# haesungpyun/seoul_tourism_recommendation_NGCF

Measured on AMD Instinct MI355X. Metric: NGCF 3-layer forward: propagated edges/sec + achieved HBM GB/s, d=128, higher is better.
Workload: dtype f32

## Files before the change

seoul_tourism_recommendation_ngcf_amd/csrc/common.h:

```cpp
#ifndef NGCF_COMMON_H
#define NGCF_COMMON_H

#include <hip/hip_runtime.h>

#include <algorithm>
#include <cstdarg>
#include <cstdint>
#include <cstdio>
#include <cstdlib>
#include <cstring>
#include <numeric>
#include <thread>
#include <vector>

#include "../../include/ngcf_hip.h"

inline thread_local char g_err[512] = "";

inline int fail(int code, const char *fmt, ...)
{
    va_list ap;
    va_start(ap, fmt);
    vsnprintf(g_err, sizeof(g_err), fmt, ap);
    va_end(ap);
    return code;
}

#define HIP_TRY(expr)                                                                          \
    do {                                                                                       \
        hipError_t e_ = (expr);                                                                \
        if (e_ != hipSuccess)                                                                  \
            return fail(NGCF_ERR_HIP, "%s failed: %s (%s:%d)", #expr, hipGetErrorString(e_),   \
                        __FILE__, __LINE__);                                                   \
    } while (0)

#define LAUNCH_CHECK()                                                                         \
    do {                                                                                       \
        hipError_t e_ = hipGetLastError();                                                     \
        if (e_ != hipSuccess)                                                                  \
            return fail(NGCF_ERR_HIP, "kernel launch failed: %s (%s:%d)", hipGetErrorString(e_), \
                        __FILE__, __LINE__);                                                   \
    } while (0)


struct NgcfOptions {
    int no_fork = 0;
    int no_slicing = 0;
    int no_ldstab = 0;
    int no_panel_split = 0;
    int no_tail_table = 0;
    int no_pad_product = 0;
    int64_t fork_min = 200000000;
    int dense_direct = 1;
    int dense_resident = 1;
    int dense_resident_min_rows = 106496;
    int dense_small_tiles = 1;
    int dense_tall = 1;
    int dense_il_lab = 0;
    int t_rows_bitmap = 1;
    int bwd_input_resident = 1;
    int slice_max_mb = 48;
    int swept_lpe = 16;
    int swept_waves = 0;
    int swept_cut = 4;
    int swept_no_moments = 0;
    int swept_order_rows = 0;
    int swept_debug = 0;
    int swept_window_kb = 0;
    int swept_spin = 500;
    int swept_lead = -2;
    int swept_sync_every = 1;
    int swept_prio_kb = 256;
    int swept_prio_graded = 1;
    int swept_nt = 0;
    int swept_merge = 0;
    char swept_trace[480] = "";
};
extern NgcfOptions g_opts;
const NgcfOptions &ngcf_opts();


constexpr int kMaxDevices = 64;
inline int current_device_slot()
{
    int dev = 0;
    if (hipGetDevice(&dev) != hipSuccess || dev < 0) dev = 0;
    return dev % kMaxDevices;
}

inline int64_t align_up(int64_t x, int64_t a) { return (x + a - 1) / a * a; }
inline bool aligned16(const void *p) { return (reinterpret_cast<uintptr_t>(p) & 15) == 0; }


inline int grid_for(int64_t n, int block)

{
    int64_t g = (n + block - 1) / block;
    if (g < 1) g = 1;
    if (g > 256 * 16) g = 256 * 16;
    return (int)g;
}



struct ngcf_csr {
    int64_t n_rows = 0, n_cols = 0, nnz = 0;
    int64_t max_row_len = 0;
    int64_t *rowptr = nullptr;
    int32_t *colidx = nullptr;
    float *vals = nullptr;
    bool owns = false;
    int64_t cap = 0, pos_len = 0;
    int32_t *pos = nullptr;
    int32_t *scan_blk = nullptr;
    bool borrows_plan = false;
    const struct ngcf_csr *filter_src = nullptr;
    int32_t seg_len = 0;
    int64_t n_seg = 0, n_heavy = 0;
    int32_t *seg_row = nullptr;
    int64_t *seg_begin = nullptr;
    int32_t *heavy_row = nullptr;
    int64_t *heavy_seg_ptr = nullptr;
    struct RowGroup {
        int64_t begin, end;
        bool sliceable;
        int32_t col_lo, col_hi;
        bool lds_table = false;
    };
    std::vector<RowGroup> groups;
    int mode = 0;
    struct SegSet {
        int64_t n_seg = 0, n_heavy = 0;
        int32_t *seg_row = nullptr;
        int64_t *seg_begin = nullptr;
        int32_t *heavy_row = nullptr;
        int64_t *heavy_seg_ptr = nullptr;
    };
    struct Swept {
        struct Part {
            int64_t row_lo = 0, row_hi = 0;
            int waves = 0, rows_per_wave = 0;
            int lpe = 16;
            int32_t n_rowpass = 0, n_win = 0, win_cols = 0, col_lo = 0, col_hi = 0;
            int64_t n_slots = 0, n_partial = 0, n_heavy = 0, partial_base = 0;
            int64_t *tptr = nullptr;
            int32_t *e_pack = nullptr;
            float *e_val = nullptr;
            int32_t *dst = nullptr;
            int32_t *prow = nullptr;
            int32_t *heavy_row = nullptr;
            int64_t *heavy_seg_ptr = nullptr;
        };
        std::vector<Part> parts;
        std::vector<char> group_swept;
        SegSet out;
        int64_t n_partial = 0;
        uint32_t *barrier = nullptr;
        mutable hipStream_t barrier_owner[4] = {nullptr, nullptr, nullptr, nullptr};
        mutable int barrier_used = 0;
        int built_mode = 0;
        int lpe = 16;
    } swept;
};


static const int32_t kLdsTableRows = 512;
static const int32_t kDefaultSegLen = 2048;
static inline int32_t default_seg_len(int64_t nnz)
{
    int32_t s = 64;
    while (s < kDefaultSegLen && (int64_t)s * 4096 < nnz) s *= 2;
    return s;
}

void free_swept(ngcf_csr *c);
int build_swept_plan(ngcf_csr *c, hipStream_t stream);
bool swept_usable(const ngcf_csr *c, int64_t ldE, int d);
void prof_mark(hipStream_t stream, int which);

__device__ inline uint32_t mix32(uint64_t x)
{
    x ^= x >> 33;
    x *= 0xff51afd7ed558ccdULL;
    x ^= x >> 33;
    x *= 0xc4ceb9fe1a85ec53ULL;
    x ^= x >> 33;
    return (uint32_t)x;
}

constexpr uint64_t kSeedPtrTag = 0xD5EDull;
__device__ inline uint64_t resolve_seed(uint64_t s)
{
    if ((s >> 48) == kSeedPtrTag) s = *reinterpret_cast<const uint64_t *>(s & 0xFFFFFFFFFFFFull);
    const uint32_t lo = __builtin_amdgcn_readfirstlane((uint32_t)s), hi = __builtin_amdgcn_readfirstlane((uint32_t)(s >> 32));
    return ((uint64_t)hi << 32) | lo;
}

struct EdgeDrop {
    int n;
    uint32_t thr;
    uint64_t seed[4];
    int transposed;
};

struct EdgeDropR {
    int n;
    uint32_t thr;
// ... 100 lines not shown
```

seoul_tourism_recommendation_ngcf_amd/csrc/dense.hip:

```cpp
#include "common.h"
#include <type_traits>

#ifndef NGCF_DC
#define NGCF_DC 16
#endif
#define NGCF_KC (2 * NGCF_DC)

typedef float f32x16 __attribute__((ext_vector_type(16)));
typedef float f32x4 __attribute__((ext_vector_type(4)));

__global__ __launch_bounds__(256) void pack_weights_kernel(const float *__restrict__ W1, const float *__restrict__ b1,
                                                           const float *__restrict__ W2, const float *__restrict__ b2, int d_in,
                                                           int d_out, int n_chunks, int DOP, int NT, float *__restrict__ Wt,
                                                           float *__restrict__ bias2)
{
    __shared__ float tile[NGCF_KC][33];
    const int groups = DOP / 32;
    const int chunk = blockIdx.x / groups, g = blockIdx.x % groups;
    for (int idx = threadIdx.x; idx < 32 * NGCF_KC; idx += 256) {
        const int w = idx / NGCF_KC, kl = idx % NGCF_KC;
        const int within = g * 32 + w;
        const int t = within % NT, j = (within / NT) % 32, cw = within / (NT * 32);
        const int oc = (cw * NT + t) * 32 + j;
        const int col = chunk * NGCF_DC + (kl % NGCF_DC);
// ... 230 lines not shown
#pragma unroll
        for (int r = 0; r < 16; ++r) {
            const int lr = rw * 32 + (r & 3) + 8 * (r >> 2) + 4 * lh;
            float s = 0.f;
#pragma unroll
            for (int q = 0; q < CW; ++q) s += ssq[lr * CW + q];
            rowss[r] = s;
        }
    }
    if (row0 + BM <= n_rows && d_out == WCOLS) {
#pragma unroll
        for (int r = 0; r < 16; ++r) {
            const int64_t grow = row0 + rw * 32 + (r & 3) + 8 * (r >> 2) + 4 * lh;
            const float inv = 1.f / fmaxf(sqrtf(rowss[r]), 1e-12f);
            float *nrow = norm + grow * ldn + cw * NT * 32 + li;
#pragma unroll
            for (int t = 0; t < NT; ++t) nrow[t * 32] = acc[t][r] * inv;
        }
        if (carry) {
#pragma unroll
            for (int r = 0; r < 16; ++r) {
                const int64_t grow = row0 + rw * 32 + (r & 3) + 8 * (r >> 2) + 4 * lh;
                float *crow = carry + grow * ldc + cw * NT * 32 + li;
#pragma unroll
                for (int t = 0; t < NT; ++t) crow[t * 32] = acc[t][r];
            }
        }
        return;
    }
#pragma unroll
    for (int r = 0; r < 16; ++r) {
        const int64_t grow = row0 + rw * 32 + (r & 3) + 8 * (r >> 2) + 4 * lh;
        if (grow >= n_rows) continue;
        const float nrm = fmaxf(sqrtf(rowss[r]), 1e-12f);
        const float inv = 1.f / nrm;
#pragma unroll
        for (int t = 0; t < NT; ++t) {
            const int col = (cw * NT + t) * 32 + li;
            if (col < d_out) {
                const float v = acc[t][r];
                if (carry) carry[grow * ldc + col] = v;
                norm[grow * ldn + col] = v * inv;
            }
        }
    }
}

constexpr int kResWaves = 8, kResWGs = 256;

__global__ __launch_bounds__(kResWaves * 64) void layer_dense_resident_kernel(
    const float *__restrict__ LE, int64_t ldLE, const float *__restrict__ Es, int64_t ldE, int64_t n_rows, int d_in, int d_out,
    const float *__restrict__ Wt, const float *__restrict__ bias2, int n_chunks, float leaky, float drop_p, uint64_t drop_seed_in,
    const float *__restrict__ drop_mask, int64_t ldm, float *__restrict__ carry, int64_t ldc, float *__restrict__ norm, int64_t ldn)
{
    const uint64_t drop_seed = drop_p > 0.f ? resolve_seed(drop_seed_in) : drop_seed_in;
    constexpr int NT = 4, WCOLS = 128;
    extern __shared__ float Wres[];
    const int tid = threadIdx.x, wave = tid >> 6, lane = tid & 63;
    const int li = lane & 31, lh = lane >> 5;
    {
        const f32x4 *src = reinterpret_cast<const f32x4 *>(Wt);
        f32x4 *dst = reinterpret_cast<f32x4 *>(Wres);
        const int n4 = n_chunks * NGCF_KC * WCOLS / 4;
        for (int i = tid; i < n4; i += kResWaves * 64) dst[i] = src[i];
    }
    __syncthreads();
    const int64_t n_tiles = (n_rows + 31) / 32;
    const int d4 = (d_in + 3) & ~3;
    const float *W = Wres + li * NT;
    float bz[NT];
#pragma unroll
    for (int t = 0; t < NT; ++t) bz[t] = bias2[t * 32 + li];
    const int last = n_chunks - 1;
    const int64_t tile_step = (int64_t)gridDim.x * kResWaves;
    auto row_of = [&](int64_t t) {
        int64_t g = t * 32 + li;
        return g < n_rows ? g : n_rows - 1;
    };
    auto fetch = [&](const float *le_row, const float *e_row, int c, f32x4 &la, f32x4 &lb, f32x4 &ea, f32x4 &eb) {
        const int ca = c * NGCF_DC + lh * 4, cb = ca + 8;
        const int cca = ca < d4 ? ca : d4 - 4, ccb = cb < d4 ? cb : d4 - 4;
        la = *reinterpret_cast<const f32x4 *>(le_row + cca);
        ea = *reinterpret_cast<const f32x4 *>(e_row + cca);
        lb = *reinterpret_cast<const f32x4 *>(le_row + ccb);
        eb = *reinterpret_cast<const f32x4 *>(e_row + ccb);
    };
    f32x4 la0, lb0, ea0, eb0, la1, lb1, ea1, eb1;
    int64_t tile = (int64_t)blockIdx.x * kResWaves + wave;
    {
        const int64_t g0 = row_of(tile < n_tiles ? tile : 0);
        fetch(LE + g0 * ldLE, Es + g0 * ldE, 0, la0, lb0, ea0, eb0);
        fetch(LE + g0 * ldLE, Es + g0 * ldE, last < 1 ? last : 1, la1, lb1, ea1, eb1);
    }
    for (; tile < n_tiles; tile += tile_step) {
        const int64_t row0 = tile * 32;
        const int64_t grow_l = row_of(tile);
        const float *le_row = LE + grow_l * ldLE, *e_row = Es + grow_l * ldE;
        f32x16 acc[NT];
#pragma unroll
        for (int t = 0; t < NT; ++t)
#pragma unroll
            for (int r = 0; r < 16; ++r) acc[t][r] = 0.f;
        auto form = [&](int c, f32x4 la, f32x4 lb, f32x4 ea, f32x4 eb, f32x4 (&a4)[4]) {
            const int ca = c * NGCF_DC + lh * 4, cb = ca + 8;
            if (cb + 4 > d_in) {
#pragma unroll
                for (int q = 0; q < 4; ++q) {
                    if (ca + q >= d_in) la[q] = 0.f, ea[q] = 0.f;
                    if (cb + q >= d_in) lb[q] = 0.f, eb[q] = 0.f;
                }
            }
            a4[0] = la + ea, a4[1] = lb + eb, a4[2] = la * ea, a4[3] = lb * eb;
        };
        auto chunk_mfma = [&](int c, const f32x4 (&a4)[4]) {
            const float *wc = W + (int64_t)c * NGCF_KC * WCOLS;
#pragma unroll
            for (int kb = 0; kb < 4; ++kb) {
#pragma unroll
                for (int sx = 0; sx < 4; ++sx) {
                    const f32x4 bv = *reinterpret_cast<const f32x4 *>(wc + (kb * 8 + lh * 4 + sx) * WCOLS);
                    acc[0] = __builtin_amdgcn_mfma_f32_32x32x2f32(a4[kb][sx], bv.x, acc[0], 0, 0, 0);
                    acc[1] = __builtin_amdgcn_mfma_f32_32x32x2f32(a4[kb][sx], bv.y, acc[1], 0, 0, 0);
                    acc[2] = __builtin_amdgcn_mfma_f32_32x32x2f32(a4[kb][sx], bv.z, acc[2], 0, 0, 0);
                    acc[3] = __builtin_amdgcn_mfma_f32_32x32x2f32(a4[kb][sx], bv.w, acc[3], 0, 0, 0);
                }
            }
        };
        int c = 0;
        for (; c + 1 < n_chunks; c += 2) {
            {
                f32x4 a4[4];
                form(c, la0, lb0, ea0, eb0, a4);
                fetch(le_row, e_row, c + 2 < last ? c + 2 : last, la0, lb0, ea0, eb0);
                __builtin_amdgcn_sched_barrier(0);
                chunk_mfma(c, a4);
            }
            {
                f32x4 a4[4];
                form(c + 1, la1, lb1, ea1, eb1, a4);
                fetch(le_row, e_row, c + 3 < last ? c + 3 : last, la1, lb1, ea1, eb1);
                __builtin_amdgcn_sched_barrier(0);
                chunk_mfma(c + 1, a4);
            }
        }
        if (c < n_chunks) {
            f32x4 a4[4];
            form(c, la0, lb0, ea0, eb0, a4);
            chunk_mfma(c, a4);
        }
        {
            const int64_t gn = row_of(tile + tile_step < n_tiles ? tile + tile_step : tile);
            fetch(LE + gn * ldLE, Es + gn * ldE, 0, la0, lb0, ea0, eb0);
            fetch(LE + gn * ldLE, Es + gn * ldE, last < 1 ? last : 1, la1, lb1, ea1, eb1);
            __builtin_amdgcn_sched_barrier(0);
        }
        const float keep_scale = drop_p > 0.f ? 1.f / (1.f - drop_p) : 1.f;
        const uint32_t drop_thr = drop_p > 0.f ? (uint32_t)((double)drop_p * 4294967296.0) : 0u;
        float rowss[16];
#pragma unroll
        for (int r = 0; r < 16; ++r) rowss[r] = 0.f;
        const bool any_drop = drop_mask || drop_p > 0.f;
        if (!any_drop) {
#pragma unroll
            for (int t = 0; t < NT; ++t)
#pragma unroll
                for (int r = 0; r < 16; ++r) {
                    float v = acc[t][r] + bz[t];
                    v = v >= 0.f ? v : leaky * v;
                    acc[t][r] = v;
                    rowss[r] = fmaf(v, v, rowss[r]);
                }
        } else {
#pragma unroll
            for (int t = 0; t < NT; ++t) {
                const int col = t * 32 + li;
#pragma unroll
                for (int r = 0; r < 16; ++r) {
                    float v = acc[t][r] + bz[t];
                    v = v >= 0.f ? v : leaky * v;
                    const int64_t grow = row0 + (r & 3) + 8 * (r >> 2) + 4 * lh;
                    if (drop_mask) v *= (grow < n_rows && col < d_out) ? drop_mask[grow * ldm + col] : 0.f;
                    else {
                        const uint32_t h = mix32(drop_seed ^ ((uint64_t)grow * 0x9E3779B97F4A7C15ULL + (uint64_t)col));
                        v = h < drop_thr ? 0.f : v * keep_scale;
                    }
                    acc[t][r] = v;
                    rowss[r] = fmaf(v, v, rowss[r]);
                }
            }
        }
#pragma unroll
        for (int r = 0; r < 16; ++r) {
            float s2 = rowss[r];
            s2 += __shfl_xor(s2, 1);
            s2 += __shfl_xor(s2, 2);
            s2 += __shfl_xor(s2, 4);
            s2 += __shfl_xor(s2, 8);
            s2 += __shfl_xor(s2, 16);
            rowss[r] = s2;
        }
        if (row0 + 32 <= n_rows && d_out == WCOLS) {
#pragma unroll
            for (int r = 0; r < 16; ++r) {
                const int64_t grow = row0 + (r & 3) + 8 * (r >> 2) + 4 * lh;
                const float inv = 1.f / fmaxf(sqrtf(rowss[r]), 1e-12f);
                float *nrow = norm + grow * ldn + li;
#pragma unroll
                for (int t = 0; t < NT; ++t) nrow[t * 32] = acc[t][r] * inv;
            }
            if (carry) {
#pragma unroll
                for (int r = 0; r < 16; ++r) {
                    float *crow = carry + (row0 + (r & 3) + 8 * (r >> 2) + 4 * lh) * ldc + li;
#pragma unroll
                    for (int t = 0; t < NT; ++t) crow[t * 32] = acc[t][r];
                }
            }
            continue;
        }
#pragma unroll
        for (int r = 0; r < 16; ++r) {
            const int64_t grow = row0 + (r & 3) + 8 * (r >> 2) + 4 * lh;
            if (grow >= n_rows) continue;
            const float inv = 1.f / fmaxf(sqrtf(rowss[r]), 1e-12f);
#pragma unroll
            for (int t = 0; t < NT; ++t) {
                const int col = t * 32 + li;
                if (col < d_out) {
                    const float v = acc[t][r];
                    if (carry) carry[grow * ldc + col] = v;
                    norm[grow * ldn + col] = v * inv;
                }
            }
        }
    }
}

#ifdef NGCF_LAB
__global__ __launch_bounds__(kResWaves * 64) void layer_dense_resident2_kernel(
    const float *__restrict__ LE, int64_t ldLE, const float *__restrict__ Es, int64_t ldE, int64_t n_rows, int d_in, int d_out,
    const float *__restrict__ Wt, const float *__restrict__ bias2, int n_chunks, float leaky, float drop_p, uint64_t drop_seed_in,
    const float *__restrict__ drop_mask, int64_t ldm, float *__restrict__ carry, int64_t ldc, float *__restrict__ norm, int64_t ldn)
{
    const uint64_t drop_seed = drop_p > 0.f ? resolve_seed(drop_seed_in) : drop_seed_in;
    constexpr int NT = 4, WCOLS = 128, TP = 2;
    extern __shared__ float Wres[];
    const int tid = threadIdx.x, wave = tid >> 6, lane = tid & 63;
    const int li = lane & 31, lh = lane >> 5;
    {
        const f32x4 *src = reinterpret_cast<const f32x4 *>(Wt);
        f32x4 *dst = reinterpret_cast<f32x4 *>(Wres);
        const int n4 = n_chunks * NGCF_KC * WCOLS / 4;
        for (int i = tid; i < n4; i += kResWaves * 64) dst[i] = src[i];
    }
    __syncthreads();
    const int64_t n_pairs = (n_rows + 32 * TP - 1) / (32 * TP);
    const int d4 = (d_in + 3) & ~3;
    const float *W = Wres + li * NT + lh * 4 * WCOLS;
    float bz[NT];
#pragma unroll
    for (int t = 0; t < NT; ++t) bz[t] = bias2[t * 32 + li];
    const int last = n_chunks - 1;
    const int64_t pair_step = (int64_t)gridDim.x * kResWaves;
    auto row_of = [&](int64_t pr, int u) {
        int64_t g = pr * (32 * TP) + u * 32 + li;
        return g < n_rows ? g : n_rows - 1;
    };
    auto fetch = [&](const float *le_row, const float *e_row, int c, f32x4 &la, f32x4 &lb, f32x4 &ea, f32x4 &eb) {
        const int ca = c * NGCF_DC + lh * 4, cb = ca + 8;
        const int cca = ca < d4 ? ca : d4 - 4, ccb = cb < d4 ? cb : d4 - 4;
        la = *reinterpret_cast<const f32x4 *>(le_row + cca);
        ea = *reinterpret_cast<const f32x4 *>(e_row + cca);
        lb = *reinterpret_cast<const f32x4 *>(le_row + ccb);
        eb = *reinterpret_cast<const f32x4 *>(e_row + ccb);
    };
    f32x4 la[TP], lb[TP], ea[TP], eb[TP];
    int64_t pair = (int64_t)blockIdx.x * kResWaves + wave;
#pragma unroll
    for (int u = 0; u < TP; ++u) {
        const int64_t g0 = row_of(pair < n_pairs ? pair : 0, u);
        fetch(LE + g0 * ldLE, Es + g0 * ldE, 0, la[u], lb[u], ea[u], eb[u]);
    }
    for (; pair < n_pairs; pair += pair_step) {
        const int64_t row0 = pair * (32 * TP);
        const float *le_row[TP], *e_row[TP];
#pragma unroll
        for (int u = 0; u < TP; ++u) {
            const int64_t g = row_of(pair, u);
            le_row[u] = LE + g * ldLE, e_row[u] = Es + g * ldE;
        }
        f32x16 acc[TP][NT];
#pragma unroll
        for (int u = 0; u < TP; ++u)
#pragma unroll
            for (int t = 0; t < NT; ++t)
#pragma unroll
                for (int r = 0; r < 16; ++r) acc[u][t][r] = 0.f;
        for (int c = 0; c < n_chunks; ++c) {
            f32x4 a4[TP][4];
            const int ca = c * NGCF_DC + lh * 4, cb = ca + 8;
#pragma unroll
            for (int u = 0; u < TP; ++u) {
                if (cb + 4 > d_in) {
#pragma unroll
                    for (int q = 0; q < 4; ++q) {
                        if (ca + q >= d_in) la[u][q] = 0.f, ea[u][q] = 0.f;
// ... 583 lines not shown
#pragma unroll
        for (int kb = 0; kb < 4; ++kb) b[kb] = *reinterpret_cast<const f32x4 *>(w + kb * 256);
    };
    f32x16 acc[MT];
#pragma unroll
    for (int m = 0; m < MT; ++m)
#pragma unroll
        for (int r = 0; r < 16; ++r) acc[m][r] = 0.f;
    const float *xs_r = Xs + li * XLD + lh * 4;
    auto read_a = [&](int buf, int kb, f32x4 (&a)[MT]) {
#pragma unroll
        for (int m = 0; m < MT; ++m)
            a[m] = *reinterpret_cast<const f32x4 *>(xs_r + buf * XBUF + m * 32 * XLD + (kb >> 1) * NGCF_DC + (kb & 1) * 8);
    };
    auto cl = [&](int c) { return c < last ? c : last; };
    f32x4 an[MT];
    auto step = [&](int c, int buf, const f32x4 (&b)[4], XRegs &x) {
        f32x4 a0[MT], a1[MT];
#pragma unroll
        for (int m = 0; m < MT; ++m) a0[m] = an[m];
#pragma unroll
        for (int kb = 0; kb < 4; kb += 2) {
            read_a(buf, kb + 1, a1);
            __builtin_amdgcn_sched_barrier(0);
#pragma unroll
            for (int sx = 0; sx < 4; ++sx)
#pragma unroll
                for (int m = 0; m < MT; ++m) acc[m] = __builtin_amdgcn_mfma_f32_32x32x2f32(a0[m][sx], b[kb][sx], acc[m], 0, 0, 0);
            if (kb + 2 < 4) read_a(buf, kb + 2, a0);
            else {
                const int b2 = buf >= 1 ? buf - 1 : 2;
                if constexpr (!(LAB & 2)) {
                    store_x(cl(c + 2), b2, x);
                    load_x(cl(c + 4), x);
                }
                read_a(buf == 2 ? 0 : buf + 1, 0, an);
            }
            __builtin_amdgcn_sched_barrier(0);
#pragma unroll
            for (int sx = 0; sx < 4; ++sx)
#pragma unroll
                for (int m = 0; m < MT; ++m) acc[m] = __builtin_amdgcn_mfma_f32_32x32x2f32(a1[m][sx], b[kb + 1][sx], acc[m], 0, 0, 0);
        }
    };
    load_x(0, x0);
    load_b(0, b0);
    load_x(cl(1), x1);
    load_b(cl(1), b1);
    store_x(0, 0, x0);
    load_x(cl(2), x0);
    store_x(cl(1), 1, x1);
    load_x(cl(3), x1);
    __syncthreads();
    read_a(0, 0, an);
    int buf = 0;
    int c = 0;
    for (; c + 1 < n_chunks; c += 2) {
        step(c, buf, b0, x0);
        if constexpr (!(LAB & 4)) load_b(cl(c + 2), b0);
        if constexpr (!(LAB & 1)) __syncthreads();
        buf = buf == 2 ? 0 : buf + 1;
        step(c + 1, buf, b1, x1);
        if constexpr (!(LAB & 4)) load_b(cl(c + 3), b1);
        if constexpr (!(LAB & 1)) __syncthreads();
        buf = buf == 2 ? 0 : buf + 1;
    }
    if (c < n_chunks) step(c, buf, b0, x0);
    const float keep_scale = drop_p > 0.f ? 1.f / (1.f - drop_p) : 1.f;
    const uint32_t drop_thr = drop_p > 0.f ? (uint32_t)((double)drop_p * 4294967296.0) : 0u;
    const int col = ct * 32 + li;
    const float bz = bias2[col];
    if (col >= d_out) return;
#pragma unroll
    for (int m = 0; m < MT; ++m)
#pragma unroll
        for (int r = 0; r < 16; ++r) {
            const int64_t grow = row0 + m * 32 + (r & 3) + 8 * (r >> 2) + 4 * lh;
            if (grow >= n_rows) continue;
            float v = acc[m][r] + bz;
            v = v >= 0.f ? v : leaky * v;
            if (drop_mask) v *= drop_mask[grow * ldm + col];
            else if (drop_p > 0.f) {
                const uint32_t h = mix32(drop_seed ^ ((uint64_t)grow * 0x9E3779B97F4A7C15ULL + (uint64_t)col));
                v = h < drop_thr ? 0.f : v * keep_scale;
            }
            if (carry) carry[grow * ldc + col] = v;
            norm[grow * ldn + col] = v;
        }
}

template <int CW>
__global__ __launch_bounds__(256) void row_scale_kernel(float *__restrict__ norm, int64_t ldn, int64_t n_rows, int d_out)
{
    const int lane = threadIdx.x & 63, li = lane & 31, half = lane >> 5;
    const int64_t row = (int64_t)blockIdx.x * 4 + (threadIdx.x >> 6);
    if (row >= n_rows) return;
    float *x = norm + row * ldn;
    constexpr int PP = CW / 2;
    float v[PP][4], part[PP];
#pragma unroll
    for (int p = 0; p < PP; ++p) {
        const int cw = half + 2 * p;
        float s = 0.f;
#pragma unroll
        for (int t = 0; t < 4; ++t) {
            const int col = cw * 128 + t * 32 + li;
            v[p][t] = col < d_out ? x[col] : 0.f;
            s = fmaf(v[p][t], v[p][t], s);
        }
        s += __shfl_xor(s, 1);
        s += __shfl_xor(s, 2);
        s += __shfl_xor(s, 4);
        s += __shfl_xor(s, 8);
        s += __shfl_xor(s, 16);
        part[p] = s;
    }
    float other[PP];
#pragma unroll
    for (int p = 0; p < PP; ++p) other[p] = __shfl_xor(part[p], 32);
    float ss = 0.f;
#pragma unroll
    for (int p = 0; p < PP; ++p) {
        const float even = half == 0 ? part[p] : other[p], odd = half == 0 ? other[p] : part[p];
        ss += even;
        ss += odd;
    }
    const float inv = 1.f / fmaxf(sqrtf(ss), 1e-12f);
#pragma unroll
    for (int p = 0; p < PP; ++p)
#pragma unroll
        for (int t = 0; t < 4; ++t) {
            const int col = (half + 2 * p) * 128 + t * 32 + li;
            if (col < d_out) x[col] = v[p][t] * inv;
        }
}

static int dense_dop(int d_out)
{
    if (d_out <= 32) return 32;
    if (d_out <= 64) return 64;
    if (d_out <= 96) return 96;
    if (d_out <= 128) return 128;
    if (d_out <= 256) return 256;
    if (d_out <= 512) return 512;
    return -1;
}

extern "C" int64_t ngcf_dense_workspace_bytes(int d_in, int d_out)
{
    int dop = dense_dop(d_out);
    if (dop < 0 || d_in <= 0) return -1;
    dop = std::max(dop, 128);
    const int64_t n_chunks = (d_in + NGCF_DC - 1) / NGCF_DC;
    return align_up((n_chunks * NGCF_KC * dop + dop) * (int64_t)sizeof(float), 256) + 256;
}

template <int RW, int CW, int NT>
static int launch_dense(bool al, int64_t n_rows, const float *LE, int64_t ldLE, const float *Es, int64_t ldE, int d_in,
                        int d_out, const float *Wt, const float *bias2, int n_chunks, float leaky, float drop_p,
                        uint64_t seed, const float *drop_mask, int64_t ldm, float *carry, int64_t ldc, float *norm, int64_t ldn,
                        hipStream_t stream)
{
    const int64_t blocks = (n_rows + 32 * RW - 1) / (32 * RW);
    if (blocks == 0) return NGCF_OK;
    if (al && ldLE >= align_up(d_in, 4) && ldE >= align_up(d_in, 4) && d_in >= 4)
        layer_dense_kernel<RW, CW, NT, true, true><<<dim3((unsigned)blocks), 256, 0, stream>>>(
            LE, ldLE, Es, ldE, n_rows, d_in, d_out, Wt, bias2, n_chunks, leaky, drop_p, seed, drop_mask, ldm, carry, ldc, norm, ldn);
    else if (al)
        layer_dense_kernel<RW, CW, NT, true, false><<<dim3((unsigned)blocks), 256, 0, stream>>>(
            LE, ldLE, Es, ldE, n_rows, d_in, d_out, Wt, bias2, n_chunks, leaky, drop_p, seed, drop_mask, ldm, carry, ldc, norm, ldn);
    else
        layer_dense_kernel<RW, CW, NT, false, false><<<dim3((unsigned)blocks), 256, 0, stream>>>(
            LE, ldLE, Es, ldE, n_rows, d_in, d_out, Wt, bias2, n_chunks, leaky, drop_p, seed, drop_mask, ldm, carry, ldc, norm, ldn);
    LAUNCH_CHECK();
    return NGCF_OK;
}

extern "C" int ngcf_layer_dense_f32(const float *LE, int64_t ldLE, const float *Es, int64_t ldEs, int64_t n_rows,
                                    int d_in, const float *W1, const float *b1, const float *W2, const float *b2,
                                    int d_out, float leaky, float drop_p, uint64_t drop_seed, const float *drop_mask,
                                    int64_t ld_mask, float *carry, int64_t ldc, float *norm, int64_t ldn, void *workspace,
                                    int64_t workspace_bytes, void *stream_)
{
    hipStream_t stream = (hipStream_t)stream_;
    if (!LE || !Es || !W1 || !b1 || !W2 || !b2 || !norm) return fail(NGCF_ERR_ARG, "layer_dense: null argument");
    if (n_rows < 0 || d_in <= 0 || d_out <= 0) return fail(NGCF_ERR_ARG, "layer_dense: bad sizes");
    int dop = dense_dop(d_out);
    if (dop < 0) return fail(NGCF_ERR_ARG, "layer_dense: d_out=%d > 512 is not supported", d_out);
    const bool small_rows = dop <= 128 && n_rows <= 16384 && ngcf_opts().dense_small_tiles;
    if (small_rows) dop = 128;
    if (!(drop_p >= 0.f && drop_p < 1.f)) return fail(NGCF_ERR_ARG, "layer_dense: drop_p=%f not in [0,1)", drop_p);
    if (ldLE < d_in || ldEs < d_in || ldn < d_out || (carry && ldc < d_out) || (drop_mask && ld_mask < d_out))
        return fail(NGCF_ERR_ARG, "layer_dense: leading dimension too small");
    const int64_t need = ngcf_dense_workspace_bytes(d_in, d_out);
    if (!workspace || workspace_bytes < need)
        return fail(NGCF_ERR_WORKSPACE, "layer_dense: workspace %lld B < %lld B", (long long)workspace_bytes, (long long)need);
    const int n_chunks = (d_in + NGCF_DC - 1) / NGCF_DC;
    float *Wt = reinterpret_cast<float *>(align_up((int64_t)(uintptr_t)workspace, 256));
    float *bias2 = Wt + (int64_t)n_chunks * NGCF_KC * dop;
    const bool al = (ldLE % 4 == 0) && (ldEs % 4 == 0) && aligned16(LE) && aligned16(Es);
    const int direct_env = ngcf_opts().dense_direct;
    const bool direct = direct_env && dop >= 256 && al && ldLE >= align_up(d_in, 4) && ldEs >= align_up(d_in, 4) && d_in >= 4 &&
                        n_rows > 0 && (n_rows <= 8192 || direct_env == 2);
    const int tall_env = ngcf_opts().dense_tall;
    const bool tall_pays = dop == 512 ? (n_rows <= 6144 || n_rows > 8192) : (n_rows > 8192 && n_rows <= 131072);
    if (tall_env && dop >= 256 && al && ldLE >= align_up(d_in, 4) && ldEs >= align_up(d_in, 4) && d_in >= 4 && n_rows > 0 &&
        (tall_pays || tall_env == 2)) {
        const int n_ct = dop / 32;
        pack_weights_tall_kernel<<<dim3((unsigned)(n_chunks * n_ct)), 256, 0, stream>>>(W1, b1, W2, b2, d_in, d_out, dop, Wt, bias2);
        LAUNCH_CHECK();
        const int64_t groups = (n_rows + kTallRows - 1) / kTallRows;
#define NGCF_TALL(L) \
    layer_dense_tall_kernel<L><<<dim3((unsigned)(groups * (n_ct / 4))), 256, 0, stream>>>( \
        LE, ldLE, Es, ldEs, n_rows, d_in, d_out, Wt, bias2, n_chunks, n_ct, leaky, drop_p, drop_seed, drop_mask, ld_mask, carry, ldc, norm, ldn)
#ifdef NGCF_LAB
        switch (ngcf_opts().dense_il_lab) {
        case 1: NGCF_TALL(1); break;
        case 2: NGCF_TALL(2); break;
        case 3: NGCF_TALL(3); break;
        case 4: NGCF_TALL(4); break;
        case 7: NGCF_TALL(7); break;
        default: NGCF_TALL(0); break;
        }
#else
        NGCF_TALL(0);
#endif
#undef NGCF_TALL
        LAUNCH_CHECK();
        if (dop == 256) row_scale_kernel<2><<<dim3((unsigned)((n_rows + 3) / 4)), 256, 0, stream>>>(norm, ldn, n_rows, d_out);
        else row_scale_kernel<4><<<dim3((unsigned)((n_rows + 3) / 4)), 256, 0, stream>>>(norm, ldn, n_rows, d_out);
        LAUNCH_CHECK();
        return NGCF_OK;
    }
    pack_weights_kernel<<<dim3((unsigned)(n_chunks * (dop / 32))), 256, 0, stream>>>(W1, b1, W2, b2, d_in, d_out, n_chunks, dop,
                                                                                    small_rows ? 1 : dop <= 128 ? dop / 32 : 4, Wt, bias2);
    LAUNCH_CHECK();
#define NGCF_DENSE(RW, CW, NT) \
    return launch_dense<RW, CW, NT>(al, n_rows, LE, ldLE, Es, ldEs, d_in, d_out, Wt, bias2, n_chunks, leaky, drop_p, \
                                    drop_seed, drop_mask, ld_mask, carry, ldc, norm, ldn, stream)
    {
        const int resident = ngcf_opts().dense_resident;
        const int64_t lds_bytes = (int64_t)n_chunks * NGCF_KC * 128 * (int64_t)sizeof(float);
        if (resident && dop == 128 && al && ldLE >= align_up(d_in, 4) && ldEs >= align_up(d_in, 4) && d_in >= 4 &&
            lds_bytes <= 150 * 1024 && n_rows >= (int64_t)ngcf_opts().dense_resident_min_rows) {
            static bool attr_set[kMaxDevices] = {};
            const int dev_i = current_device_slot();
            if (!attr_set[dev_i]) {
                HIP_TRY(hipFuncSetAttribute(reinterpret_cast<const void *>(layer_dense_resident_kernel),
                                            hipFuncAttributeMaxDynamicSharedMemorySize, 160 * 1024));
                attr_set[dev_i] = true;
            }
#ifdef NGCF_LAB
            if (resident == 3) {
                static bool r2_set = false;
                if (!r2_set) {
                    (void)hipFuncSetAttribute(reinterpret_cast<const void *>(layer_dense_resident2_kernel), hipFuncAttributeMaxDynamicSharedMemorySize, 160 * 1024);
                    r2_set = true;
                }
                layer_dense_resident2_kernel<<<dim3(kResWGs), kResWaves * 64, (size_t)lds_bytes, stream>>>(
                    LE, ldLE, Es, ldEs, n_rows, d_in, d_out, Wt, bias2, n_chunks, leaky, drop_p, drop_seed, drop_mask, ld_mask, carry, ldc,
                    norm, ldn);
                LAUNCH_CHECK();
                return NGCF_OK;
            }
#endif
#ifdef NGCF_LAB
            if (resident == 2 && d_out == 128 && (n_chunks == 8 || n_chunks == 9) && ldn < (1 << 24) && ldc < (1 << 24) && ldn % 4 == 0 &&
                aligned16(norm) && (!carry || (ldc % 4 == 0 && aligned16(carry)))) {
                const int64_t il_lds = lds_bytes + kIlWaves * 2048;
#define NGCF_IL(NCH, CARRY) \
    do { \
        static bool il_set[kMaxDevices] = {}; \
        if (!il_set[dev_i]) { \
            HIP_TRY(hipFuncSetAttribute(reinterpret_cast<const void *>(layer_dense_resident_il_kernel<NCH, CARRY>), \
                                        hipFuncAttributeMaxDynamicSharedMemorySize, 160 * 1024)); \
            il_set[dev_i] = true; \
        } \
        layer_dense_resident_il_kernel<NCH, CARRY><<<dim3(kResWGs), kIlWaves * 64, (size_t)il_lds, stream>>>( \
            LE, ldLE, Es, ldEs, n_rows, d_in, d_out, Wt, bias2, leaky, drop_p, drop_seed, drop_mask, ld_mask, carry, ldc, norm, ldn); \
    } while (0)
#define NGCF_IL_LAB(L) \
    layer_dense_resident_il_kernel<8, true, L><<<dim3(kResWGs), kIlWaves * 64, (size_t)il_lds, stream>>>( \
        LE, ldLE, Es, ldEs, n_rows, d_in, d_out, Wt, bias2, leaky, drop_p, drop_seed, drop_mask, ld_mask, carry, ldc, norm, ldn)
                if (const int lab = ngcf_opts().dense_il_lab; lab && n_chunks == 8 && carry) {
                    static bool lab_set = false;
                    if (!lab_set) {
                        (void)hipFuncSetAttribute(reinterpret_cast<const void *>(layer_dense_resident_il_kernel<8, true, 1>), hipFuncAttributeMaxDynamicSharedMemorySize, 160 * 1024);
                        (void)hipFuncSetAttribute(reinterpret_cast<const void *>(layer_dense_resident_il_kernel<8, true, 2>), hipFuncAttributeMaxDynamicSharedMemorySize, 160 * 1024);
                        (void)hipFuncSetAttribute(reinterpret_cast<const void *>(layer_dense_resident_il_kernel<8, true, 3>), hipFuncAttributeMaxDynamicSharedMemorySize, 160 * 1024);
                        (void)hipFuncSetAttribute(reinterpret_cast<const void *>(layer_dense_resident_il_kernel<8, true, 6>), hipFuncAttributeMaxDynamicSharedMemorySize, 160 * 1024);
                        (void)hipFuncSetAttribute(reinterpret_cast<const void *>(layer_dense_resident_il_kernel<8, true, 10>), hipFuncAttributeMaxDynamicSharedMemorySize, 160 * 1024);
                        lab_set = true;
                    }
                    switch (lab) {
                    case 1: NGCF_IL_LAB(1); break;
                    case 2: NGCF_IL_LAB(2); break;
                    case 3: NGCF_IL_LAB(3); break;
                    case 6: NGCF_IL_LAB(6); break;
                    default: NGCF_IL_LAB(10); break;
                    }
                    LAUNCH_CHECK();
                    return NGCF_OK;
                }
#undef NGCF_IL_LAB
                if (n_chunks == 8) { if (carry) NGCF_IL(8, true); else NGCF_IL(8, false); }
                else { if (carry) NGCF_IL(9, true); else NGCF_IL(9, false); }
#undef NGCF_IL
                LAUNCH_CHECK();
                return NGCF_OK;
            }
#endif
            layer_dense_resident_kernel<<<dim3(kResWGs), kResWaves * 64, (size_t)lds_bytes, stream>>>(
                LE, ldLE, Es, ldEs, n_rows, d_in, d_out, Wt, bias2, n_chunks, leaky, drop_p, drop_seed, drop_mask, ld_mask, carry, ldc,
                norm, ldn);
            LAUNCH_CHECK();
            return NGCF_OK;
        }
    }
    if (direct) {
        const int64_t blocks = (n_rows + 31) / 32;
        if (dop == 256)
            layer_dense_direct_kernel<2, 4><<<dim3((unsigned)blocks), 128, 0, stream>>>(
                LE, ldLE, Es, ldEs, n_rows, d_in, d_out, Wt, bias2, n_chunks, leaky, drop_p, drop_seed, drop_mask, ld_mask, carry, ldc,
                norm, ldn);
        else
            layer_dense_direct_kernel<4, 4><<<dim3((unsigned)blocks), 256, 0, stream>>>(
                LE, ldLE, Es, ldEs, n_rows, d_in, d_out, Wt, bias2, n_chunks, leaky, drop_p, drop_seed, drop_mask, ld_mask, carry, ldc,
                norm, ldn);
        LAUNCH_CHECK();
        return NGCF_OK;
    }
    if (small_rows) NGCF_DENSE(1, 4, 1);
    switch (dop) {
    case 32: NGCF_DENSE(4, 1, 1);
    case 64: NGCF_DENSE(4, 1, 2);
    case 96: NGCF_DENSE(4, 1, 3);
    case 128: NGCF_DENSE(4, 1, 4);
    case 256: NGCF_DENSE(2, 2, 4);
    default: NGCF_DENSE(1, 4, 4);
    }
#undef NGCF_DENSE
}

extern "C" int64_t ngcf_layer_workspace_bytes(const ngcf_csr_t *c, int d_in, int d_out)
{
    if (!c) return -1;
    const int64_t a = ngcf_spmm_workspace_bytes(c, d_in);
    const int64_t b = ngcf_dense_workspace_bytes(d_in, d_out);
    if (a < 0 || b < 0) return -1;
    const int64_t le = align_up(c->n_rows * align_up(d_in, 32) * (int64_t)sizeof(float), 256);
    return a + b + le + 256;
}

extern "C" int ngcf_layer_fused_f32(const ngcf_csr_t *c, const float *Eg, int64_t ldEg, const float *Es, int64_t ldEs,
                                    int d_in, const float *W1, const float *b1, const float *W2, const float *b2,
                                    int d_out, float leaky, float drop_p, uint64_t drop_seed, const float *drop_mask,
                                    int64_t ld_mask, float *carry, int64_t ldc, float *norm, int64_t ldn, void *workspace,
                                    int64_t workspace_bytes, void *stream)
{
    if (!c) return fail(NGCF_ERR_ARG, "layer_fused: null csr");
    const int64_t need = ngcf_layer_workspace_bytes(c, d_in, d_out);
    if (need < 0) return fail(NGCF_ERR_ARG, "layer_fused: unsupported widths d_in=%d d_out=%d", d_in, d_out);
    if (!workspace || workspace_bytes < need)
        return fail(NGCF_ERR_WORKSPACE, "layer_fused: workspace %lld B < %lld B", (long long)workspace_bytes, (long long)need);
    char *ws = reinterpret_cast<char *>(align_up((int64_t)(uintptr_t)workspace, 256));
    const int64_t ldLE = align_up(d_in, 32);
    float *LE = reinterpret_cast<float *>(ws);
    ws += align_up(c->n_rows * ldLE * (int64_t)sizeof(float), 256);
    const int64_t spmm_ws = ngcf_spmm_workspace_bytes(c, d_in);
    void *ws_spmm = ws;
    ws += spmm_ws;
    const int64_t dense_ws = ngcf_dense_workspace_bytes(d_in, d_out);
    void *ws_dense = ws;
    const int d_sp = ngcf_spmm_product_width(c, Eg, ldEg, d_in);
    int rc = ngcf_spmm_csr_f32(c, Eg, ldEg, d_sp, LE, ldLE, ws_spmm, spmm_ws, stream);
    if (rc != NGCF_OK) return rc;
    return ngcf_layer_dense_f32(LE, ldLE, Es, ldEs, c->n_rows, d_in, W1, b1, W2, b2, d_out, leaky, drop_p, drop_seed,
                                drop_mask, ld_mask, carry, ldc, norm, ldn, ws_dense, dense_ws, stream);
}
```

Before: 27.71 billion.

## Add bf16x3 split-precision MFMA dense kernel and make it default

```diff
diff --git a/seoul_tourism_recommendation_ngcf_amd/csrc/common.h b/seoul_tourism_recommendation_ngcf_amd/csrc/common.h
--- a/seoul_tourism_recommendation_ngcf_amd/csrc/common.h
+++ b/seoul_tourism_recommendation_ngcf_amd/csrc/common.h
@@ -52,7 +52,7 @@
     int no_pad_product = 0;
     int64_t fork_min = 200000000;
     int dense_direct = 1;
-    int dense_resident = 1;
+    int dense_resident = 4;
     int dense_resident_min_rows = 106496;
     int dense_small_tiles = 1;
     int dense_tall = 1;
diff --git a/seoul_tourism_recommendation_ngcf_amd/csrc/dense.hip b/seoul_tourism_recommendation_ngcf_amd/csrc/dense.hip
--- a/seoul_tourism_recommendation_ngcf_amd/csrc/dense.hip
+++ b/seoul_tourism_recommendation_ngcf_amd/csrc/dense.hip
@@ -406,6 +406,238 @@
             const int64_t gn = row_of(tile + tile_step < n_tiles ? tile + tile_step : tile);
             fetch(LE + gn * ldLE, Es + gn * ldE, 0, la0, lb0, ea0, eb0);
             fetch(LE + gn * ldLE, Es + gn * ldE, last < 1 ? last : 1, la1, lb1, ea1, eb1);
+            __builtin_amdgcn_sched_barrier(0);
+        }
+        const float keep_scale = drop_p > 0.f ? 1.f / (1.f - drop_p) : 1.f;
+        const uint32_t drop_thr = drop_p > 0.f ? (uint32_t)((double)drop_p * 4294967296.0) : 0u;
+        float rowss[16];
+#pragma unroll
+        for (int r = 0; r < 16; ++r) rowss[r] = 0.f;
+        const bool any_drop = drop_mask || drop_p > 0.f;
+        if (!any_drop) {
+#pragma unroll
+            for (int t = 0; t < NT; ++t)
+#pragma unroll
+                for (int r = 0; r < 16; ++r) {
+                    float v = acc[t][r] + bz[t];
+                    v = v >= 0.f ? v : leaky * v;
+                    acc[t][r] = v;
+                    rowss[r] = fmaf(v, v, rowss[r]);
+                }
+        } else {
+#pragma unroll
+            for (int t = 0; t < NT; ++t) {
+                const int col = t * 32 + li;
+#pragma unroll
+                for (int r = 0; r < 16; ++r) {
+                    float v = acc[t][r] + bz[t];
+                    v = v >= 0.f ? v : leaky * v;
+                    const int64_t grow = row0 + (r & 3) + 8 * (r >> 2) + 4 * lh;
+                    if (drop_mask) v *= (grow < n_rows && col < d_out) ? drop_mask[grow * ldm + col] : 0.f;
+                    else {
+                        const uint32_t h = mix32(drop_seed ^ ((uint64_t)grow * 0x9E3779B97F4A7C15ULL + (uint64_t)col));
+                        v = h < drop_thr ? 0.f : v * keep_scale;
+                    }
+                    acc[t][r] = v;
+                    rowss[r] = fmaf(v, v, rowss[r]);
+                }
+            }
+        }
+#pragma unroll
+        for (int r = 0; r < 16; ++r) {
+            float s2 = rowss[r];
+            s2 += __shfl_xor(s2, 1);
+            s2 += __shfl_xor(s2, 2);
+            s2 += __shfl_xor(s2, 4);
+            s2 += __shfl_xor(s2, 8);
+            s2 += __shfl_xor(s2, 16);
+            rowss[r] = s2;
+        }
+        if (row0 + 32 <= n_rows && d_out == WCOLS) {
+#pragma unroll
+            for (int r = 0; r < 16; ++r) {
+                const int64_t grow = row0 + (r & 3) + 8 * (r >> 2) + 4 * lh;
+                const float inv = 1.f / fmaxf(sqrtf(rowss[r]), 1e-12f);
+                float *nrow = norm + grow * ldn + li;
+#pragma unroll
+                for (int t = 0; t < NT; ++t) nrow[t * 32] = acc[t][r] * inv;
+            }
+            if (carry) {
+#pragma unroll
+                for (int r = 0; r < 16; ++r) {
+                    float *crow = carry + (row0 + (r & 3) + 8 * (r >> 2) + 4 * lh) * ldc + li;
+#pragma unroll
+                    for (int t = 0; t < NT; ++t) crow[t * 32] = acc[t][r];
+                }
+            }
+            continue;
+        }
+#pragma unroll
+        for (int r = 0; r < 16; ++r) {
+            const int64_t grow = row0 + (r & 3) + 8 * (r >> 2) + 4 * lh;
+            if (grow >= n_rows) continue;
+            const float inv = 1.f / fmaxf(sqrtf(rowss[r]), 1e-12f);
+#pragma unroll
+            for (int t = 0; t < NT; ++t) {
+                const int col = t * 32 + li;
+                if (col < d_out) {
+                    const float v = acc[t][r];
+                    if (carry) carry[grow * ldc + col] = v;
+                    norm[grow * ldn + col] = v * inv;
+                }
+            }
+        }
+    }
+}
+
+typedef __bf16 bf16x8 __attribute__((ext_vector_type(8)));
+typedef float f32x8 __attribute__((ext_vector_type(8)));
+
+__device__ __forceinline__ void split3(f32x8 x, bf16x8 &h, bf16x8 &m, bf16x8 &l)
+{
+    h = __builtin_convertvector(x, bf16x8);
+    const f32x8 r = x - __builtin_convertvector(h, f32x8);
+    m = __builtin_convertvector(r, bf16x8);
+    l = __builtin_convertvector(r - __builtin_convertvector(m, f32x8), bf16x8);
+}
+
+__global__ __launch_bounds__(256) void pack_weights_split_kernel(const float *__restrict__ W1, const float *__restrict__ b1,
+                                                                 const float *__restrict__ W2, const float *__restrict__ b2,
+                                                                 int d_in, int d_out, int n_chunks, bf16x8 *__restrict__ Whm,
+                                                                 bf16x8 *__restrict__ Wl, float *__restrict__ bias2)
+{
+    const int idx = blockIdx.x * 256 + threadIdx.x;
+    if (idx < n_chunks * 512) {
+        const int lane = idx & 63, frag = idx >> 6, t = frag & 3, s = (frag >> 2) & 1, c = frag >> 3;
+        const int col = t * 32 + (lane & 31), in0 = c * NGCF_DC + 8 * (lane >> 5);
+        const float *w = (s ? W2 : W1) + (int64_t)col * d_in;
+        f32x8 x;
+#pragma unroll
+        for (int j = 0; j < 8; ++j) x[j] = (col < d_out && in0 + j < d_in) ? w[in0 + j] : 0.f;
+        bf16x8 h, m, l;
+        split3(x, h, m, l);
+        Whm[(frag * 2 + 0) * 64 + lane] = h;
+        Whm[(frag * 2 + 1) * 64 + lane] = m;
+        Wl[idx] = l;
+    }
+    if (blockIdx.x == 0)
+        for (int j = threadIdx.x; j < 128; j += 256)
+            bias2[j] = j < d_out ? (b1[j] + b1[j]) + b2[j] : 0.f;
+}
+
+__global__ __launch_bounds__(kResWaves * 64) void layer_dense_split_kernel(
+    const float *__restrict__ LE, int64_t ldLE, const float *__restrict__ Es, int64_t ldE, int64_t n_rows, int d_in, int d_out,
+    const bf16x8 *__restrict__ Whm, const bf16x8 *__restrict__ Wl, const float *__restrict__ bias2, int n_chunks, float leaky,
+    float drop_p, uint64_t drop_seed_in, const float *__restrict__ drop_mask, int64_t ldm, float *__restrict__ carry, int64_t ldc,
+    float *__restrict__ norm, int64_t ldn)
+{
+    const uint64_t drop_seed = drop_p > 0.f ? resolve_seed(drop_seed_in) : drop_seed_in;
+    constexpr int NT = 4, WCOLS = 128;
+    extern __shared__ bf16x8 Wsh[];
+    const int tid = threadIdx.x, wave = tid >> 6, lane = tid & 63;
+    const int li = lane & 31, lh = lane >> 5;
+    for (int i = tid; i < n_chunks * 1024; i += kResWaves * 64) Wsh[i] = Whm[i];
+    __syncthreads();
+    const int64_t n_tiles = (n_rows + 31) / 32;
+    const int d4 = (d_in + 3) & ~3;
+    float bz[NT];
+#pragma unroll
+    for (int t = 0; t < NT; ++t) bz[t] = bias2[t * 32 + li];
+    const int last = n_chunks - 1;
+    const int64_t tile_step = (int64_t)gridDim.x * kResWaves;
+    auto row_of = [&](int64_t t) {
+        int64_t g = t * 32 + li;
+        return g < n_rows ? g : n_rows - 1;
+    };
+    auto fetch = [&](const float *le_row, const float *e_row, int c, f32x4 &la, f32x4 &lb, f32x4 &ea, f32x4 &eb) {
+        const int ca = c * NGCF_DC + lh * 8, cb = ca + 4;
+        const int cca = ca < d4 ? ca : d4 - 4, ccb = cb < d4 ? cb : d4 - 4;
+        la = *reinterpret_cast<const f32x4 *>(le_row + cca);
+        ea = *reinterpret_cast<const f32x4 *>(e_row + cca);
+        lb = *reinterpret_cast<const f32x4 *>(le_row + ccb);
+        eb = *reinterpret_cast<const f32x4 *>(e_row + ccb);
+    };
+    auto fetch_l = [&](int c, bf16x8 (&bl)[8]) {
+#pragma unroll
+        for (int f = 0; f < 8; ++f) bl[f] = Wl[(c * 8 + f) * 64 + lane];
+    };
+    f32x4 la0, lb0, ea0, eb0, la1, lb1, ea1, eb1;
+    bf16x8 bl0[8], bl1[8];
+    fetch_l(0, bl0);
+    int64_t tile = (int64_t)blockIdx.x * kResWaves + wave;
+    {
+        const int64_t g0 = row_of(tile < n_tiles ? tile : 0);
+        fetch(LE + g0 * ldLE, Es + g0 * ldE, 0, la0, lb0, ea0, eb0);
+        fetch(LE + g0 * ldLE, Es + g0 * ldE, last < 1 ? last : 1, la1, lb1, ea1, eb1);
+    }
+    for (; tile < n_tiles; tile += tile_step) {
+        const int64_t row0 = tile * 32;
+        const int64_t grow_l = row_of(tile);
+        const float *le_row = LE + grow_l * ldLE, *e_row = Es + grow_l * ldE;
+        f32x16 acc[NT];
+#pragma unroll
+        for (int t = 0; t < NT; ++t)
+#pragma unroll
+            for (int r = 0; r < 16; ++r) acc[t][r] = 0.f;
+        auto form = [&](int c, f32x4 la, f32x4 lb, f32x4 ea, f32x4 eb, bf16x8 (&a)[2][3]) {
+            const int ca = c * NGCF_DC + lh * 8, cb = ca + 4;
+            if (cb + 4 > d_in) {
+#pragma unroll
+                for (int q = 0; q < 4; ++q) {
+                    if (ca + q >= d_in) la[q] = 0.f, ea[q] = 0.f;
+                    if (cb + q >= d_in) lb[q] = 0.f, eb[q] = 0.f;
+                }
+            }
+            const f32x4 sa = la + ea, sb = lb + eb, pa = la * ea, pb = lb * eb;
+            split3(__builtin_shufflevector(sa, sb, 0, 1, 2, 3, 4, 5, 6, 7), a[0][0], a[0][1], a[0][2]);
+            split3(__builtin_shufflevector(pa, pb, 0, 1, 2, 3, 4, 5, 6, 7), a[1][0], a[1][1], a[1][2]);
+        };
+        auto chunk_mfma = [&](int c, const bf16x8 (&a)[2][3], const bf16x8 (&bl)[8]) {
+            const bf16x8 *wc = Wsh + c * 1024 + lane;
+#pragma unroll
+            for (int s = 0; s < 2; ++s) {
+                const bf16x8 &ah = a[s][0], &am = a[s][1], &al = a[s][2];
+#pragma unroll
+                for (int t = 0; t < NT; ++t) {
+                    const bf16x8 bh = wc[((s * 4 + t) * 2 + 0) * 64], bm = wc[((s * 4 + t) * 2 + 1) * 64];
+                    acc[t] = __builtin_amdgcn_mfma_f32_32x32x16_bf16(am, bm, acc[t], 0, 0, 0);
+                    acc[t] = __builtin_amdgcn_mfma_f32_32x32x16_bf16(al, bh, acc[t], 0, 0, 0);
+                    acc[t] = __builtin_amdgcn_mfma_f32_32x32x16_bf16(ah, bl[s * 4 + t], acc[t], 0, 0, 0);
+                    acc[t] = __builtin_amdgcn_mfma_f32_32x32x16_bf16(am, bh, acc[t], 0, 0, 0);
+                    acc[t] = __builtin_amdgcn_mfma_f32_32x32x16_bf16(ah, bm, acc[t], 0, 0, 0);
+                    acc[t] = __builtin_amdgcn_mfma_f32_32x32x16_bf16(ah, bh, acc[t], 0, 0, 0);
+                }
+            }
+        };
+        int c = 0;
+        for (; c + 1 < n_chunks; c += 2) {
+            {
+                bf16x8 a[2][3];
+                form(c, la0, lb0, ea0, eb0, a);
+                fetch(le_row, e_row, c + 2 < last ? c + 2 : last, la0, lb0, ea0, eb0);
+                fetch_l(c + 1, bl1);
+                __builtin_amdgcn_sched_barrier(0);
+                chunk_mfma(c, a, bl0);
+            }
+            {
+                bf16x8 a[2][3];
+                form(c + 1, la1, lb1, ea1, eb1, a);
+                fetch(le_row, e_row, c + 3 < last ? c + 3 : last, la1, lb1, ea1, eb1);
+                fetch_l(c + 2 < last ? c + 2 : last, bl0);
+                __builtin_amdgcn_sched_barrier(0);
+                chunk_mfma(c + 1, a, bl1);
+            }
+        }
+        if (c < n_chunks) {
+            bf16x8 a[2][3];
+            form(c, la0, lb0, ea0, eb0, a);
+            chunk_mfma(c, a, bl0);
+        }
+        {
+            const int64_t gn = row_of(tile + tile_step < n_tiles ? tile + tile_step : tile);
+            fetch(LE + gn * ldLE, Es + gn * ldE, 0, la0, lb0, ea0, eb0);
+            fetch(LE + gn * ldLE, Es + gn * ldE, last < 1 ? last : 1, la1, lb1, ea1, eb1);
+            fetch_l(0, bl0);
             __builtin_amdgcn_sched_barrier(0);
         }
         const float keep_scale = drop_p > 0.f ? 1.f / (1.f - drop_p) : 1.f;
@@ -1295,7 +1527,9 @@
     if (dop < 0 || d_in <= 0) return -1;
     dop = std::max(dop, 128);
     const int64_t n_chunks = (d_in + NGCF_DC - 1) / NGCF_DC;
-    return align_up((n_chunks * NGCF_KC * dop + dop) * (int64_t)sizeof(float), 256) + 256;
+    const int64_t fp32_packed = (n_chunks * NGCF_KC * dop + dop) * (int64_t)sizeof(float);
+    const int64_t split_packed = 128 * (int64_t)sizeof(float) + n_chunks * 3 * 8 * 1024;
+    return align_up(std::max(fp32_packed, split_packed), 256) + 256;
 }
 
 template <int RW, int CW, int NT>
@@ -1375,9 +1609,11 @@
         LAUNCH_CHECK();
         return NGCF_OK;
     }
-    pack_weights_kernel<<<dim3((unsigned)(n_chunks * (dop / 32))), 256, 0, stream>>>(W1, b1, W2, b2, d_in, d_out, n_chunks, dop,
-                                                                                    small_rows ? 1 : dop <= 128 ? dop / 32 : 4, Wt, bias2);
-    LAUNCH_CHECK();
+    auto pack_fp32 = [&]() {
+        pack_weights_kernel<<<dim3((unsigned)(n_chunks * (dop / 32))), 256, 0, stream>>>(W1, b1, W2, b2, d_in, d_out, n_chunks, dop,
+                                                                                        small_rows ? 1 : dop <= 128 ? dop / 32 : 4, Wt, bias2);
+        return hipGetLastError();
+    };
 #define NGCF_DENSE(RW, CW, NT) \
     return launch_dense<RW, CW, NT>(al, n_rows, LE, ldLE, Es, ldEs, d_in, d_out, Wt, bias2, n_chunks, leaky, drop_p, \
                                     drop_seed, drop_mask, ld_mask, carry, ldc, norm, ldn, stream)
@@ -1388,6 +1624,26 @@
             lds_bytes <= 150 * 1024 && n_rows >= (int64_t)ngcf_opts().dense_resident_min_rows) {
             static bool attr_set[kMaxDevices] = {};
             const int dev_i = current_device_slot();
+            if (resident == 4) {
+                static bool split_set[kMaxDevices] = {};
+                if (!split_set[dev_i]) {
+                    HIP_TRY(hipFuncSetAttribute(reinterpret_cast<const void *>(layer_dense_split_kernel),
+                                                hipFuncAttributeMaxDynamicSharedMemorySize, 160 * 1024));
+                    split_set[dev_i] = true;
+                }
+                float *sbias = Wt;
+                bf16x8 *whm = reinterpret_cast<bf16x8 *>(Wt + 128);
+                bf16x8 *wl = whm + (int64_t)n_chunks * 1024;
+                pack_weights_split_kernel<<<dim3((unsigned)(n_chunks * 2)), 256, 0, stream>>>(W1, b1, W2, b2, d_in, d_out, n_chunks,
+                                                                                              whm, wl, sbias);
+                LAUNCH_CHECK();
+                layer_dense_split_kernel<<<dim3(kResWGs), kResWaves * 64, (size_t)n_chunks * 16 * 1024, stream>>>(
+                    LE, ldLE, Es, ldEs, n_rows, d_in, d_out, whm, wl, sbias, n_chunks, leaky, drop_p, drop_seed, drop_mask, ld_mask,
+                    carry, ldc, norm, ldn);
+                LAUNCH_CHECK();
+                return NGCF_OK;
+            }
+            HIP_TRY(pack_fp32());
             if (!attr_set[dev_i]) {
                 HIP_TRY(hipFuncSetAttribute(reinterpret_cast<const void *>(layer_dense_resident_kernel),
                                             hipFuncAttributeMaxDynamicSharedMemorySize, 160 * 1024));
@@ -1460,6 +1716,7 @@
             return NGCF_OK;
         }
     }
+    HIP_TRY(pack_fp32());
     if (direct) {
         const int64_t blocks = (n_rows + 31) / 32;
         if (dop == 256)
```

Result: faster. 28.34 billion, median of 6 (+2.3%).
